# happyjin/Gaussian_process

Measured on AMD Instinct MI355X. Metric: GP-fit+predict sec and achieved fp64 TFLOP/s, N=65536 d=8, 1/2/4/8 MI355X, higher is better.
Workload: dtype f64; 1 GPU; GP fit+predict N=65536 d=8 n_test=4096 (BASELINE configs[2]); N=65536, d=8, n_test=4096, partition=single GPU

## Files before the change

gaussian_process_amd/csrc/gemm_dma.hip:

```cpp
#include <algorithm>
#include <cstdlib>
#include <type_traits>

#include "gpmi_internal.h"
#include "gpmi_plan.h"
#include <atomic>
#include <mutex>

namespace gpmi {

typedef double d4 __attribute__((ext_vector_type(4)));
typedef double d2 __attribute__((ext_vector_type(2)));

#define GPMI_LDS __attribute__((address_space(3)))
#define GPMI_GLB __attribute__((address_space(1)))
#define GPMI_CONST __attribute__((address_space(4)))

struct GemmDmaDev {
    double* C;
    const double* A;
    const double* B;
    int64_t ldc, lda, ldb;
    int Tm, Tn;
    int nchunks;
    int lower;
    int64_t diag_off;
    const int32_t* row_ncols;
    int row_block_tiles;
    const int64_t* b_block_off;
    int b_block_tiles;
    int S, logS, SM, SN, tri, nsuper;
    int pair;
    int sprefix[DMA_MAX_SM + 1];
    unsigned long long* stamps;
    int dbg;
    struct PersistSlot* slot;
    int nblocks;
};

struct PersistSlot {
    unsigned ctr[8];
    unsigned done;
    unsigned pad[7];
};

template <class PT>
__device__ __forceinline__ bool dma_block_to_tile(const PT& p, int b, int& ti, int& tj) {
    return plan_block_to_tile(p, b, ti, tj);
}

__device__ __forceinline__ bool dma_map_tile(const GemmDmaDev& p, int& ti, int& tj) {
    return dma_block_to_tile(p, blockIdx.x, ti, tj);
}

constexpr int DMA_TM = PLAN_TILE, DMA_TN = PLAN_TILE;
template <class PT>
__device__ __forceinline__ bool dma_tile_live(const PT& p, int ti, int tj) {
    return plan_tile_live(p, ti, tj, p.row_ncols);
}
constexpr int DMA_STAGE_SLOTS = (DMA_TM + DMA_TN) * 8;
constexpr int DMA_STAGES = 3;

constexpr unsigned TICKET_NONE = 0xFFFFFFFFu;

template <class PT>
__device__ __forceinline__ unsigned ticket_draw(const PT& p, int xcd) {
    const unsigned per = (unsigned)p.nblocks >> 3;
#pragma unroll 1
    for (int t = 0; t < 8; ++t) {
        const int x = (xcd + t) & 7;
        if (t && __hip_atomic_load(&p.slot->ctr[x], __ATOMIC_RELAXED, __HIP_MEMORY_SCOPE_AGENT) >= per) continue;
        const unsigned w = atomicAdd(&p.slot->ctr[x], 1u);
        if (w < per) return w * 8u + (unsigned)x;
    }
    return TICKET_NONE;
}

template <int MI, bool DBG, bool TICKET = false>
__device__ __forceinline__ void gemm_nt_dma_body(const GemmDmaDev& p) {
    constexpr int NWAVES = 16 / MI;
    constexpr int DPW = 32 / NWAVES;
    constexpr int RPW = DMA_TM / NWAVES;
    constexpr int NFR = MI + 4;
    const int dbg = DBG ? p.dbg : 0;
    extern __shared__ __attribute__((aligned(16))) char smem_raw[];
    const int tid = threadIdx.x;
    volatile GPMI_LDS int* mbox = (volatile GPMI_LDS int*)(smem_raw + DMA_STAGES * DMA_STAGE_SLOTS * 16);
    unsigned blk = blockIdx.x, nxt_blk = TICKET_NONE;
    int par = 0;
    if constexpr (TICKET) {
        if (tid == 0) mbox[0] = (int)ticket_draw(p, (int)(blockIdx.x & 7));
        __syncthreads();
        blk = (unsigned)__builtin_amdgcn_readfirstlane(mbox[0]);
        par = 1;
    }
  for (;;) {
    int ti = 0, tj = 0;
    bool live;
    if constexpr (TICKET) {
        if (blk == TICKET_NONE) break;
        live = dma_block_to_tile(p, (int)blk, ti, tj) && dma_tile_live(p, ti, tj);
        live = __builtin_amdgcn_readfirstlane(live ? 1 : 0) != 0;
        ti = __builtin_amdgcn_readfirstlane(ti);
        tj = __builtin_amdgcn_readfirstlane(tj);
    } else {
        live = dma_map_tile(p, ti, tj) && dma_tile_live(p, ti, tj);
        if (!live) return;
    }
   if (live) {
    unsigned long long st0 = 0, st1 = 0, st2 = 0, st3 = 0;
    if (DBG && (dbg & 16)) st0 = clock64();
    const int lane = tid & 63;
    const int wave = __builtin_amdgcn_readfirstlane(tid >> 6);
    const int wr = (wave >> 1) * (16 * MI);
    const int wc = (wave & 1) * 64;
    const int fr = lane & 15;
    const int fg = lane >> 4;

// ... 172 lines not shown
            if (!live) nxt_blk = ticket_draw(p, (int)(blockIdx.x & 7));
            mbox[par] = (int)nxt_blk;
        }
        __syncthreads();
        blk = (unsigned)__builtin_amdgcn_readfirstlane(mbox[par]);
        par ^= 1;
    }
  }
    if constexpr (TICKET) {
        if (tid == 0) {
            __threadfence();
            const unsigned old = atomicAdd(&p.slot->done, 1u);
            if (old == gridDim.x - 1) {
#pragma unroll
                for (int x = 0; x < 8; ++x) p.slot->ctr[x] = 0;
                p.slot->done = 0;
                __threadfence();
            }
        }
    }
}

template <int MI, bool DBG>
__global__ __launch_bounds__(1024 / MI, (MI == 4) ? 2 : 3) void gemm_nt_dma_kernel(const GemmDmaDev p) {
    gemm_nt_dma_body<MI, DBG>(p);
}

__global__ __launch_bounds__(512, 3) void chol_trailing_update_dma_kernel(const GemmDmaDev p) {
    gemm_nt_dma_body<2, false>(p);
}

constexpr int TALL_TM = 2 * DMA_TM;
constexpr int TALL_STAGE_SLOTS = (TALL_TM + DMA_TN) * 8;
constexpr int TALL_STAGES = 2;
constexpr size_t TALL_LDS = (size_t)TALL_STAGES * TALL_STAGE_SLOTS * 16;
static_assert(TALL_LDS == (size_t)DMA_STAGES * DMA_STAGE_SLOTS * 16, "the tall form keeps the LDS footprint");

template <bool DBG>
__device__ __forceinline__ void gemm_nt_dma_tall_body(const GemmDmaDev& p) {
    constexpr int DPW = 6;
    const int dbg = DBG ? p.dbg : 0;
    extern __shared__ __attribute__((aligned(16))) char smem_raw[];
    const int tid = threadIdx.x;
    int ti = 0, tj = 0;
    if (!dma_block_to_tile(p, blockIdx.x, ti, tj)) return;
    bool l0, l1;
    plan_pair_live(p, ti, tj, p.row_ncols, l0, l1);
    ti = __builtin_amdgcn_readfirstlane(ti);
    tj = __builtin_amdgcn_readfirstlane(tj);
    const bool live0 = __builtin_amdgcn_readfirstlane(l0 ? 1 : 0) != 0;
    const bool live1 = __builtin_amdgcn_readfirstlane(l1 ? 1 : 0) != 0;
    if (!live0 && !live1) return;
    unsigned long long st0 = 0, st1 = 0, st2 = 0, st3 = 0;
    if (DBG && (dbg & 16)) st0 = clock64();
    const int lane = tid & 63;
    const int wave = __builtin_amdgcn_readfirstlane(tid >> 6);
    const bool mine = (wave >> 2) ? live1 : live0;
    const int wr = (wave >> 1) * 64;
    const int wc = (wave & 1) * 64;
    const int fr = lane & 15;
    const int fg = lane >> 4;

    const int drow = lane >> 3;
    const int dkp = (lane & 7) ^ (drow & 7);
    const int arow = 32 * wave - ((ti + 1 >= p.Tm && wave >= 4) ? DMA_TM : 0);
    const double* a_row = p.A + ((int64_t)ti * DMA_TM + arow) * p.lda;
    int64_t b_row0 = (int64_t)tj * DMA_TN * p.ldb;
    if (p.b_block_off) {
        const int blk = tj / p.b_block_tiles;
        b_row0 = p.b_block_off[blk] + (int64_t)(tj - blk * p.b_block_tiles) * DMA_TN * p.ldb;
    }
    const double* b_row = p.B + b_row0 + (int64_t)(16 * wave) * p.ldb;
    const unsigned a_lane = (unsigned)((drow * p.lda + dkp * 2) * 8);
    const unsigned b_lane = (unsigned)((drow * p.ldb + dkp * 2) * 8);
    const int64_t a_step = 8 * p.lda, b_step = 8 * p.ldb;
    GPMI_LDS char* lds = (GPMI_LDS char*)smem_raw;
    const int a_dst = (32 * wave) * 128;
    const int b_dst = TALL_TM * 128 + (16 * wave) * 128;
    auto issue_dma_one = [&](int chunk, int q) {
        GPMI_LDS char* base = lds + (chunk & 1) * (TALL_STAGE_SLOTS * 16);
        const int k0 = chunk * 16;
        unsigned off = q < 4 ? a_lane : b_lane;
        asm volatile("" : "+v"(off));
        if (q < 4)
            __builtin_amdgcn_global_load_lds((const GPMI_GLB void*)((const char*)(a_row + q * a_step + k0) + off),
                                             (GPMI_LDS void*)(base + a_dst + q * 1024), 16, 0, 0);
        else
            __builtin_amdgcn_global_load_lds((const GPMI_GLB void*)((const char*)(b_row + (q - 4) * b_step + k0) + off),
                                             (GPMI_LDS void*)(base + b_dst + (q - 4) * 1024), 16, 0, 0);
    };

    const int x7 = fr & 7;
    const int sl0 = fr * 8 + (fg ^ x7);
    const int sl1 = fr * 8 + ((4 + fg) ^ x7);
    const d2* smem = reinterpret_cast<const d2*>(smem_raw);
    auto read_a = [&](int chunk, int half, int i) -> d2 {
        return smem[(chunk & 1) * TALL_STAGE_SLOTS + (wr + 16 * i) * 8 + (half ? sl1 : sl0)];
    };
    auto read_b = [&](int chunk, int half, int j) -> d2 {
        return smem[(chunk & 1) * TALL_STAGE_SLOTS + TALL_TM * 8 + (wc + 16 * j) * 8 + (half ? sl1 : sl0)];
    };

    d4 acc[4][4];
#pragma unroll
    for (int i = 0; i < 4; ++i)
#pragma unroll
        for (int j = 0; j < 4; ++j) acc[i][j] = d4{0., 0., 0., 0.};
    const int nch = p.nchunks;

#define GPMI_MFMA_X(FA, FB, T) acc[(T) >> 2][(T) & 3] = __builtin_amdgcn_mfma_f64_16x16x4f64(FA[(T) >> 2].x, FB[(T) & 3].x, acc[(T) >> 2][(T) & 3], 0, 0, 0)
#define GPMI_MFMA_Y(FA, FB, T) acc[(T) >> 2][(T) & 3] = __builtin_amdgcn_mfma_f64_16x16x4f64(FA[(T) >> 2].y, FB[(T) & 3].y, acc[(T) >> 2][(T) & 3], 0, 0, 0)
#define GPMI_FENCE() __builtin_amdgcn_sched_barrier(0)
    auto kloop = [&](auto live_tag) {
        constexpr bool LIVE = decltype(live_tag)::value;
        d2 fa[4], fb0[4], fb1[4];
#pragma unroll
        for (int q = 0; q < DPW; ++q) issue_dma_one(0, q);
        if (nch > 1) {
#pragma unroll
            for (int q = 0; q < DPW; ++q) issue_dma_one(1, q);
            asm volatile("s_waitcnt vmcnt(6)" ::: "memory");
        } else {
            asm volatile("s_waitcnt vmcnt(0)" ::: "memory");
        }
        __builtin_amdgcn_s_barrier();
        if constexpr (LIVE) {
#pragma unroll
            for (int i = 0; i < 4; ++i) fa[i] = read_a(0, 0, i);
#pragma unroll
            for (int j = 0; j < 4; ++j) fb0[j] = read_b(0, 0, j);
        }
        if (DBG && (dbg & 16)) st1 = clock64();
        auto quarter0 = [&]() {
            if constexpr (LIVE) {
#pragma unroll
                for (int t = 0; t < 16; ++t) GPMI_MFMA_X(fa, fb0, t);
                GPMI_FENCE();
            }
        };
        auto step = [&](int c) {
            const bool more2 = (c + 2 < nch) && !(dbg & 1);
            if constexpr (LIVE) {
#pragma unroll
                for (int q = 0; q < 8; ++q) {
                    GPMI_MFMA_Y(fa, fb0, 2 * q);
                    GPMI_MFMA_Y(fa, fb0, 2 * q + 1);
                    GPMI_FENCE();
                    if (q & 1) fa[q >> 1] = read_a(c, 1, q >> 1);
                    else fb1[q >> 1] = read_b(c, 1, q >> 1);
                    GPMI_FENCE();
                }
#pragma unroll
                for (int t = 0; t < 8; ++t) GPMI_MFMA_X(fa, fb1, t);
                GPMI_FENCE();
            }
            if (!(dbg & 2)) {
                asm volatile("s_waitcnt vmcnt(0)\n\ts_waitcnt lgkmcnt(0)" ::: "memory");
                __builtin_amdgcn_s_barrier();
            }
            GPMI_FENCE();
            if constexpr (LIVE) {
#pragma unroll
                for (int t = 8; t < 16; ++t) {
                    GPMI_MFMA_X(fa, fb1, t);
                    GPMI_FENCE();
                    if (more2 && t - 8 < DPW) issue_dma_one(c + 2, t - 8);
                    GPMI_FENCE();
                }
#pragma unroll
                for (int q = 0; q < 8; ++q) {
                    GPMI_MFMA_Y(fa, fb1, 2 * q);
                    GPMI_MFMA_Y(fa, fb1, 2 * q + 1);
                    GPMI_FENCE();
                    if (q & 1) fa[q >> 1] = read_a(c + 1, 0, q >> 1);
                    else fb0[q >> 1] = read_b(c + 1, 0, q >> 1);
                    GPMI_FENCE();
                }
            } else if (more2) {
#pragma unroll
                for (int q = 0; q < DPW; ++q) issue_dma_one(c + 2, q);
            }
        };
        quarter0();
        for (int c = 0; c + 1 < nch; ++c) {
            step(c);
            quarter0();
        }
        step(nch - 1);
    };
    if (mine) kloop(std::true_type{});
    else kloop(std::false_type{});
#undef GPMI_MFMA_X
#undef GPMI_MFMA_Y
#undef GPMI_FENCE
    if (!mine) return;

    if (DBG && (dbg & 16)) st2 = clock64();
    double* Cg = p.C + ((int64_t)ti * DMA_TM + wr) * p.ldc + (int64_t)tj * DMA_TN + wc;
    auto c_ptr = [&](int i, int j, int v) { return Cg + (int64_t)(16 * i + 4 * v + fg) * p.ldc + 16 * j + fr; };
    if (DBG && (dbg & 8)) {
        double t = 0.;
#pragma unroll
        for (int i = 0; i < 4; ++i)
#pragma unroll
            for (int j = 0; j < 4; ++j) t += acc[i][j][0] + acc[i][j][1] + acc[i][j][2] + acc[i][j][3];
        if (t == 123.456) Cg[0] = t;
        return;
    }
    double cv[2][4][4];
    auto load_band = [&](int i) {
#pragma unroll
        for (int j = 0; j < 4; ++j)
#pragma unroll
            for (int v = 0; v < 4; ++v) cv[i & 1][j][v] = *c_ptr(i, j, v);
    };
    auto store_band = [&](int i) {
#pragma unroll
        for (int j = 0; j < 4; ++j)
#pragma unroll
            for (int v = 0; v < 4; ++v) *c_ptr(i, j, v) = cv[i & 1][j][v] - acc[i][j][v];
    };
    load_band(0);
    if (DBG && (dbg & 16)) {
        asm volatile("s_waitcnt vmcnt(0)" ::: "memory");
        st3 = clock64();
    }
    store_band(0);
    load_band(1);
    load_band(2);
    store_band(1);
    load_band(3);
    store_band(2);
    store_band(3);
    if (DBG && (dbg & 16)) {
        asm volatile("s_waitcnt vmcnt(0)" ::: "memory");
        const unsigned long long st4 = clock64();
        if (lane == 0 && blockIdx.x < 4096) {
            unsigned long long* o = p.stamps + ((size_t)blockIdx.x * 4 + (wave & 3)) * 4;
            o[0] = st1 - st0; o[1] = st2 - st1; o[2] = st3 - st2; o[3] = st4 - st3;
        }
    }
}

template <bool DBG>
__global__ __launch_bounds__(512) __attribute__((amdgpu_num_vgpr(192))) void gemm_nt_dma_tall_kernel(const GemmDmaDev p) {
    gemm_nt_dma_tall_body<DBG>(p);
}
__global__ __launch_bounds__(512) __attribute__((amdgpu_num_vgpr(192))) void chol_trailing_update_dma256_kernel(const GemmDmaDev p) {
    gemm_nt_dma_tall_body<false>(p);
}

__global__ __launch_bounds__(512, 3) void gemm_nt_dma_ticket_kernel(const GemmDmaDev p) {
    gemm_nt_dma_body<2, false, true>(p);
}
__global__ __launch_bounds__(512, 3) void chol_trailing_update_ticket_kernel(const GemmDmaDev p) {
    gemm_nt_dma_body<2, false, true>(p);
}

template <int ROLE>
__device__ __forceinline__ void gemm_nt_dma_persist_body(const GemmDmaDev& p) {
    constexpr int MI = 2, DPW = 4, RPW = 16, NFR = 6, NT = 8, NSLOT = 4;
    constexpr int RING = DMA_STAGES * DMA_STAGE_SLOTS * 16;
    extern __shared__ __attribute__((aligned(16))) char smem_raw[];
    volatile GPMI_LDS int* mbox = (volatile GPMI_LDS int*)(smem_raw + RING);
    const int tid = threadIdx.x;
    const int lane = tid & 63;
    const int wave = __builtin_amdgcn_readfirstlane(tid >> 6);
    const int wr = (wave >> 1) * (16 * MI);
    const int wc = (wave & 1) * 64;
    const int fr = lane & 15;
    const int fg = lane >> 4;
    const int drow = lane >> 3;
    const int dkp = (lane & 7) ^ (drow & 7);
    const int xcd = blockIdx.x & 7;
    const int nch = p.nchunks;
    const int64_t ldc = p.ldc;
    GPMI_LDS char* lds = (GPMI_LDS char*)smem_raw;
    const int a_dst = (RPW * wave) * 128;
    const int b_dst = DMA_TM * 128 + (RPW * wave) * 128;
    const unsigned c_lane = (unsigned)((fg * ldc + fr) * 8);

    auto kernarg = [&]() -> const GPMI_CONST GemmDmaDev* {
        const GPMI_CONST GemmDmaDev* pp = (const GPMI_CONST GemmDmaDev*)__builtin_amdgcn_kernarg_segment_ptr();
        asm volatile("" : "+s"(pp));
        return pp;
    };
    auto uniform_ptr = [](const void* q) -> uintptr_t {
        const uintptr_t u = reinterpret_cast<uintptr_t>(q);
        const unsigned lo = (unsigned)__builtin_amdgcn_readfirstlane((int)(u & 0xffffffffu));
        const unsigned hi = (unsigned)__builtin_amdgcn_readfirstlane((int)(u >> 32));
        return ((uintptr_t)hi << 32) | lo;
    };
    struct TileRef { const double* d[DPW]; GPMI_GLB char* c; };
    auto resolve = [&](unsigned b, TileRef& t) -> bool {
        const GPMI_CONST GemmDmaDev* pp = kernarg();
        int ti, tj;
        if (!dma_block_to_tile(*pp, (int)b, ti, tj)) return false;
        if (!dma_tile_live(*pp, ti, tj)) return false;
        ti = __builtin_amdgcn_readfirstlane(ti);
        tj = __builtin_amdgcn_readfirstlane(tj);
        t.d[0] = pp->A + ((int64_t)ti * DMA_TM + RPW * wave + drow) * pp->lda + dkp * 2;
        t.d[1] = t.d[0] + 8 * pp->lda;
        int64_t b_row0 = (int64_t)tj * DMA_TN * pp->ldb;
        if (pp->b_block_off) {
            const int blk = tj / pp->b_block_tiles;
            b_row0 = pp->b_block_off[blk] + (int64_t)(tj - blk * pp->b_block_tiles) * DMA_TN * pp->ldb;
        }
        t.d[2] = pp->B + b_row0 + (int64_t)(RPW * wave + drow) * pp->ldb + dkp * 2;
        t.d[3] = t.d[2] + 8 * pp->ldb;
        double* tc = pp->C + ((int64_t)ti * DMA_TM + wr) * pp->ldc + (int64_t)tj * DMA_TN + wc;
        t.c = (GPMI_GLB char*)uniform_ptr(tc);
        return true;
    };
    auto draw = [&]() -> unsigned {
        const GPMI_CONST GemmDmaDev* pp = kernarg();
        return ticket_draw(*pp, xcd);
    };
    auto past_end = [&](unsigned b) -> bool { return b == TICKET_NONE; };
    auto scalar_flag = [](bool f) -> bool { return __builtin_amdgcn_readfirstlane(f ? 1 : 0) != 0; };
    auto draw_sync = [&](TileRef& t) -> bool {
        for (;;) {
            if (tid == 0) mbox[0] = (int)draw();
            __syncthreads();
            const unsigned w = (unsigned)__builtin_amdgcn_readfirstlane(mbox[0]);
// ... 268 lines not shown
        for (int j = 0; j < 2; ++j)
#pragma unroll
            for (int v = 0; v < 4; ++v) cv[i][j][v] = *c_ptr(i, j, v);
#pragma unroll
    for (int i = 0; i < 2; ++i)
#pragma unroll
        for (int j = 0; j < 2; ++j)
#pragma unroll
            for (int v = 0; v < 4; ++v) *c_ptr(i, j, v) = cv[i][j][v] - acc[i][j][v];
}

hipError_t launch_gemm_nt_small(hipStream_t s, const GemmArgs& a, const GemmRoute& r) {
    GemmSmallDev p;
    p.C = a.C; p.A = a.A; p.B = a.B; p.ldc = a.ldc; p.lda = a.lda; p.ldb = a.ldb;
    p.Tm = (int)(a.M / SM_T); p.Tn = (int)(a.N / SM_T); p.nchunks = (int)(a.K / 16);
    p.lower = a.lower; p.diag_off = a.diag_off;
    static PerDeviceOnce once;
    const hipError_t ea = once.run([&]() -> hipError_t {
        return hipFuncSetAttribute((const void*)gemm_nt_small_kernel<8>, hipFuncAttributeMaxDynamicSharedMemorySize, (int)(8 * GEMM_SMALL_STAGE));
    });
    if (ea != hipSuccess) return ea;
    if (r.kernel == GemmKernel::Small3) hipLaunchKernelGGL(gemm_nt_small_kernel<3>, dim3(r.grid), dim3(256), r.lds, s, p);
    else hipLaunchKernelGGL(gemm_nt_small_kernel<8>, dim3(r.grid), dim3(256), r.lds, s, p);
    return hipGetLastError();
}

struct PersistPool {
    static constexpr int SLOTS = 16384;
    PersistSlot* base = nullptr;
    int groups = 0;
    std::atomic<unsigned> head{0};
    PersistSlot* next() { return base + (head.fetch_add(1, std::memory_order_relaxed) % SLOTS); }
};

static PersistPool* persist_pool() {
    static std::mutex mu;
    static PersistPool pools[16];
    int dev = 0;
    if (hipGetDevice(&dev) != hipSuccess || dev < 0 || dev >= 16) return nullptr;
    PersistPool& pl = pools[dev];
    std::lock_guard<std::mutex> lock(mu);
    if (!pl.base) {
        hipDeviceProp_t prop;
        if (hipGetDeviceProperties(&prop, dev) != hipSuccess) return nullptr;
        void* q = nullptr;
        if (hipMalloc(&q, sizeof(PersistSlot) * PersistPool::SLOTS) != hipSuccess) return nullptr;
        if (hipMemset(q, 0, sizeof(PersistSlot) * PersistPool::SLOTS) != hipSuccess) { (void)hipFree(q); return nullptr; }
        pl.groups = (prop.multiProcessorCount / 8) * 8;
        if (pl.groups < 8) { (void)hipFree(q); return nullptr; }
        const void* fns[] = {(const void*)gemm_nt_dma_persist_kernel, (const void*)chol_trailing_update_persist_kernel,
                             (const void*)gemm_nt_dma_ticket_kernel, (const void*)chol_trailing_update_ticket_kernel};
        for (const void* f : fns)
            if (hipFuncSetAttribute(f, hipFuncAttributeMaxDynamicSharedMemorySize,
                                    (int)(DMA_STAGES * DMA_STAGE_SLOTS * 16 + 16)) != hipSuccess) { (void)hipFree(q); return nullptr; }
        pl.base = static_cast<PersistSlot*>(q);
    }
    return &pl;
}

int gemm_resident_groups() {
    const PersistPool* pool = persist_pool();
    return pool ? pool->groups : 0;
}

static_assert((size_t)DMA_STAGES * DMA_STAGE_SLOTS * 16 == GEMM_DMA_LDS && TALL_LDS == GEMM_TALL_LDS && TALL_LDS == GEMM_DMA_LDS,
              "gpmi_route.h sizes the rings of the launches; one opt-in size serves both forms");

hipError_t launch_gemm_nt_dma(hipStream_t s, const GemmArgs& a, const GemmRoute& r) {
    const TilePlan& plan = r.plan;
    GemmDmaDev p;
    p.C = a.C; p.A = a.A; p.B = a.B;
    p.ldc = a.ldc; p.lda = a.lda; p.ldb = a.ldb;
    p.Tm = plan.Tm; p.Tn = plan.Tn;
    p.nchunks = (int)(a.K / 16);
    p.lower = a.lower; p.diag_off = a.diag_off;
    p.row_ncols = a.row_ncols; p.row_block_tiles = plan.row_block_tiles;
    p.b_block_off = a.b_block_off;
    p.b_block_tiles = a.b_block_off ? (int)(a.b_block_rows / 128) : 1;
    p.S = plan.S; p.logS = plan.logS; p.SM = plan.SM; p.SN = plan.SN; p.tri = plan.tri; p.nsuper = plan.nsuper;
    p.pair = plan.pair;
    if (plan.tri == 2) std::copy(plan.sprefix, plan.sprefix + plan.SM + 1, p.sprefix);
    p.dbg = tuning().gemm_dbg & 0xff;
    p.stamps = tuning().gemm_stamps;
    p.slot = nullptr;
    p.nblocks = plan.nblocks;
    static PerDeviceOnce once;
    const hipError_t ea = once.run([&]() -> hipError_t {
        const void* fns[] = {(const void*)gemm_nt_dma_kernel<4, false>, (const void*)gemm_nt_dma_kernel<4, true>,
                             (const void*)gemm_nt_dma_kernel<2, false>, (const void*)gemm_nt_dma_kernel<2, true>,
                             (const void*)chol_trailing_update_dma_kernel, (const void*)gemm_nt_dma_tall_kernel<false>,
                             (const void*)gemm_nt_dma_tall_kernel<true>, (const void*)chol_trailing_update_dma256_kernel};
        for (const void* f : fns) {
            const hipError_t e = hipFuncSetAttribute(f, hipFuncAttributeMaxDynamicSharedMemorySize, (int)GEMM_DMA_LDS);
            if (e != hipSuccess) return e;
        }
        return hipSuccess;
    });
    if (ea != hipSuccess) return ea;
    if (r.kernel >= GemmKernel::Persist) {
        PersistPool* pool = persist_pool();
        if (!pool) return hipErrorInvalidValue;
        p.slot = pool->next();
    }
    const dim3 grid(r.grid);
    switch (r.kernel) {
        case GemmKernel::Ticket: hipLaunchKernelGGL(gemm_nt_dma_ticket_kernel, grid, dim3(512), r.lds, s, p); break;
        case GemmKernel::TicketTrail: hipLaunchKernelGGL(chol_trailing_update_ticket_kernel, grid, dim3(512), r.lds, s, p); break;
        case GemmKernel::Persist: hipLaunchKernelGGL(gemm_nt_dma_persist_kernel, grid, dim3(512), r.lds, s, p); break;
        case GemmKernel::PersistTrail: hipLaunchKernelGGL(chol_trailing_update_persist_kernel, grid, dim3(512), r.lds, s, p); break;
        case GemmKernel::Tall: hipLaunchKernelGGL(gemm_nt_dma_tall_kernel<false>, grid, dim3(512), r.lds, s, p); break;
        case GemmKernel::TallProbe: hipLaunchKernelGGL(gemm_nt_dma_tall_kernel<true>, grid, dim3(512), r.lds, s, p); break;
        case GemmKernel::TallTrail: hipLaunchKernelGGL(chol_trailing_update_dma256_kernel, grid, dim3(512), r.lds, s, p); break;
        case GemmKernel::Dma8: hipLaunchKernelGGL((gemm_nt_dma_kernel<2, false>), grid, dim3(512), r.lds, s, p); break;
        case GemmKernel::Dma8Probe: hipLaunchKernelGGL((gemm_nt_dma_kernel<2, true>), grid, dim3(512), r.lds, s, p); break;
        case GemmKernel::Dma8Trail: hipLaunchKernelGGL(chol_trailing_update_dma_kernel, grid, dim3(512), r.lds, s, p); break;
        case GemmKernel::Dma4: hipLaunchKernelGGL((gemm_nt_dma_kernel<4, false>), grid, dim3(256), r.lds, s, p); break;
        case GemmKernel::Dma4Probe: hipLaunchKernelGGL((gemm_nt_dma_kernel<4, true>), grid, dim3(256), r.lds, s, p); break;
        default: return hipErrorInvalidValue;
    }
    return hipGetLastError();
}

}
```

gaussian_process_amd/csrc/gpmi_api.hip:

```cpp
#include "gpmi_ctx.h"

using namespace gpmi;

namespace gpmi {
thread_local std::string g_err;

static thread_local Tuning t_dev_tuning;
static thread_local const Tuning* t_tuning = nullptr;
const Tuning& tuning() { return t_tuning ? *t_tuning : t_dev_tuning; }
TuneScope::TuneScope(const Tuning* t) : prev(t_tuning) { t_tuning = t; }
TuneScope::~TuneScope() { t_tuning = prev; }
static thread_local Sharing t_sharing;
Sharing& sharing() { return t_sharing; }

int ard_rescale_train(gpmi_ctx* c) {
    if (!c->ard()) return GPMI_OK;
    HIP_TRY(c->Xz.ensure((size_t)c->N * c->d * 8));
    HIP_TRY(launch_scale_inputs(c->stream, c->X.as<double>(), c->ard_rdev.as<double>(), c->N, c->d, c->Xz.as<double>()));
    HIP_TRY(hipStreamSynchronize(c->stream));
    box_scale(c->boxX, c->ard_r, c->boxZ);
    return GPMI_OK;
}
int ard_rescale_test(gpmi_ctx* c) {
    if (!c->ard()) return GPMI_OK;
// ... 15 lines not shown
    int n = 0;
    hipError_t e = hipGetDeviceCount(&n);
    if (e != hipSuccess) { *count = 0; return fail_runtime(e, "hipGetDeviceCount"); }
    *count = n;
    return GPMI_OK;
}

int gpmi_ctx_create(int device, gpmi_ctx** out) {
    if (!out) return fail_arg("gpmi_ctx_create: null out pointer");
    *out = nullptr;
    int n = 0;
    HIP_TRY(hipGetDeviceCount(&n));
    if (device < 0 || device >= n) return fail_arg("gpmi_ctx_create: no such device");
    HIP_TRY(hipSetDevice(device));
    gpmi_ctx* c = new gpmi_ctx();
    c->device = device;
    int prio_lo = 0, prio_hi = 0;
    (void)hipDeviceGetStreamPriorityRange(&prio_lo, &prio_hi);
    hipError_t e = hipStreamCreateWithPriority(&c->stream, hipStreamNonBlocking, prio_lo);
    if (e != hipSuccess) { delete c; return fail_runtime(e, "hipStreamCreate"); }
    e = hipStreamCreateWithPriority(&c->pstream, hipStreamNonBlocking, prio_hi);
    if (e != hipSuccess) { (void)hipStreamDestroy(c->stream); delete c; return fail_runtime(e, "hipStreamCreate"); }
    const char* env;
    if ((env = getenv("GPMI_NB"))) c->nb = std::max<int64_t>(128, atoll(env) / 128 * 128);
    if ((env = getenv("GPMI_LD_PAD"))) c->ld_pad = std::max<int64_t>(0, atoll(env) / 2 * 2);
    if ((env = getenv("GPMI_LOOKAHEAD"))) c->lookahead = atoi(env) ? 1 : 0;
    *out = c;
    return GPMI_OK;
}

int gpmi_ctx_destroy(gpmi_ctx* c) {
    if (!c) return GPMI_OK;
    for (gpmi_ctx* l : c->lane_ctx) (void)gpmi_ctx_destroy(l);
    c->lane_ctx.clear();
    (void)hipSetDevice(c->device);
    (void)hipStreamSynchronize(c->stream);
    for (DevBuf* b : {&c->X, &c->y, &c->A, &c->info, &c->red, &c->Xs, &c->V, &c->P, &c->vec, &c->dense,
                       &c->U, &c->Kn, &c->gpart, &c->cov_a, &c->cov_b, &c->cov_out, &c->flag, &c->vside,
                       &c->Xz, &c->Xsz, &c->ard_rdev, &c->gsum, &c->app, &c->spareA, &c->rem, &c->lap, &c->lap_part, &c->lap_out, &c->sm, &c->sm_part, &c->sm_E, &c->sm_B, &c->sm_out, &c->loov, &c->loow,
                       &c->sp_Zraw, &c->sp_Z, &c->sp_L, &c->sp_B, &c->sp_W, &c->sp_q, &c->sp_vec, &c->sp_part, &c->sp_scr, &c->sp_info, &c->sp_pred,
                       &c->sp_g0, &c->sp_g1, &c->sp_g2, &c->sp_gE, &c->sp_gpart, &c->sp_gvec})
        b->release();
    for (auto e : c->ev_pool) (void)hipEventDestroy(e);
    (void)hipStreamDestroy(c->stream);
    (void)hipStreamDestroy(c->pstream);
    delete c;
    return GPMI_OK;
}

static int set_tuning_option(Tuning& t, const char* name, int64_t value) {
    if (!strcmp(name, "gemm_small_tiles")) {
        t.gemm_small_tiles = value ? 1 : 0;
    } else if (!strcmp(name, "trsm_wave")) {
        t.trsm_wave = value ? 1 : 0;
    } else if (!strcmp(name, "gemm_small_dma")) {
        t.gemm_small_dma = value ? 1 : 0;
    } else if (!strcmp(name, "gemm_persist")) {
        t.gemm_persist = value ? 1 : 0;
    } else if (!strcmp(name, "gemm_ticket")) {
        if (value < 0 || value > 2) return fail_arg("gemm_ticket must be 0 (off), 1 (trailing updates under lookahead) or 2 (every launch)");
        t.gemm_ticket = (int)value;
    } else if (!strcmp(name, "gemm_balance")) {
        t.gemm_balance = value ? 1 : 0;
    } else if (!strcmp(name, "trsv_vinv")) {
        if (value < 0 || value > 2) return fail_arg("trsv_vinv must be 0 (16 x 16 rounds), 1 (one launch per block) or 2 (one launch)");
        t.trsv_vinv = (int)value;
    } else if (!strcmp(name, "panel_fused")) {
        t.panel_fused = value ? 1 : 0;
    } else if (!strcmp(name, "rbf_blocks")) {
        if (value < 1 || value > (1 << 24)) return fail_arg("rbf_blocks must be in 1..2^24");
        t.rbf_blocks = (int)value;
    } else if (!strcmp(name, "gemm_dma_waves")) {
        if (value != 4 && value != 8) return fail_arg("gemm_dma_waves must be 4 or 8");
        t.gemm_dma_waves = (int)value;
    } else if (!strcmp(name, "gemm_tall")) {
        if (value < 0 || value > 1) return fail_arg("gemm_tall must be 0 (128 x 128 blocks) or 1 (256 x 128 blocks for large launches)");
        t.gemm_tall = (int)value;
    } else if (!strcmp(name, "tall_min_tiles")) {
        if (value < 0 || value > (1 << 30)) return fail_arg("tall_min_tiles must be in 0..2^30");
        t.tall_min_tiles = (int)value;
    } else if (!strcmp(name, "tall_min_tiles_slack")) {
        if (value < 0 || value > (1 << 30)) return fail_arg("tall_min_tiles_slack must be in 0..2^30");
        t.tall_min_tiles_slack = (int)value;
    } else if (!strcmp(name, "gemm_dma")) {
        t.gemm_use_dma = value ? 1 : 0;
    } else {
        return -1;
    }
    return GPMI_OK;
}

int gpmi_set_option(gpmi_ctx* c, const char* name, int64_t value) {
    if (!c || !name) return fail_arg("gpmi_set_option: null argument");
    if (!strcmp(name, "nb")) {
        if (value != 0 && (value < 128 || value % 128)) return fail_arg("nb must be 0 (auto) or a positive multiple of 128");
        c->nb = value;
    } else if (!strcmp(name, "ld_pad")) {
        if (value < 0 || value % 2) return fail_arg("ld_pad must be even and >= 0");
        c->ld_pad = value;
        c->res.drop_fit();
    } else if (!strcmp(name, "timing")) {
        c->timing = value ? 1 : 0;
    } else if (!strcmp(name, "lookahead")) {
        c->lookahead = value ? 1 : 0;
    } else if (!strcmp(name, "la_min")) {
        if (value < 0) return fail_arg("la_min must be >= 0");
        c->la_min = value;
    } else if (!strcmp(name, "shallow_min")) {
        if (value < 0) return fail_arg("shallow_min must be >= 0");
        c->shallow_min = value;
    } else if (!strcmp(name, "sparse_slab")) {
        if (value < 0) return fail_arg("sparse_slab must be >= 0 (0: by size)");
        c->sparse_slab = value;
    } else if (!strcmp(name, "reserve")) {
        if (value < 0) return fail_arg("reserve must be >= 0 (points that gpmi_append may add in place)");
        c->reserve = value;
    } else if (!strcmp(name, "append_skinny")) {
        if (value < -1 || value > 1) return fail_arg("append_skinny must be -1 (by size), 0 (never) or 1 (whenever allowed)");
        c->append_skinny = (int)value;
    } else if (!strcmp(name, "remove_keep_spare")) {
        c->remove_keep_spare = value ? 1 : 0;
        if (!c->remove_keep_spare) {
            HIP_TRY(hipSetDevice(c->device));
            c->spareA.release();
        }
    } else if (!strcmp(name, "lanes")) {
        if (value < 0 || value > 8) return fail_arg("lanes must be 0 (by size) .. 8");
        c->lanes = (int)value;
    } else {
        const int rc = set_tuning_option(c->tune, name, value);
        if (rc < 0) return fail_arg("gpmi_set_option: unknown option");
        return rc;
    }
    return GPMI_OK;
}

int gpmi_dev_set_option(const char* name, int64_t value) {
    if (!name) return fail_arg("gpmi_dev_set_option: null argument");
    const int rc = set_tuning_option(t_dev_tuning, name, value);
    if (rc < 0) return fail_arg("gpmi_dev_set_option: unknown option");
    return rc;
}

int gpmi_set_kernel(gpmi_ctx* c, int kind, double p0, double p1) {
    if (!c) return fail_arg("gpmi_set_kernel: null context");
    if (kind < 0 || kind == 3 || kind > 6)
        return fail_arg("gpmi_set_kernel: kind must be 0 (rbf), 1 (linear), 2 (periodic) or 4, 5, 6 (Matern nu = 1/2, 3/2, 5/2)");
    if (kind == 2 && (!(p0 != 0.0) || !(p1 != 0.0))) return fail_arg("gpmi_set_kernel: period and lengthscale must be non-zero");
    c->kind = kind; c->kp0 = p0; c->kp1 = p1;
    c->res.drop_fit();
    return GPMI_OK;
}

int gpmi_set_kernel_params(gpmi_ctx* c, int kind, const double* params, int nparams) {
    if (!c || !params) return fail_arg("gpmi_set_kernel_params: null argument");
    if (kind != 3) {
        if (kind < 0 || kind > 6 || nparams != 2) return fail_arg("gpmi_set_kernel_params: kinds 0-2 and 4-6 take 2 parameters");
        return gpmi_set_kernel(c, kind, params[0], params[1]);
    }
    if (nparams != 11) return fail_arg("gpmi_set_kernel_params: the CO2 composite kernel takes 11 hyper-parameters (CO2_example.py:86-89)");
    if (!(params[1] != 0.0) || !(params[3] != 0.0) || !(params[4] != 0.0) || !(params[6] != 0.0) || !(params[7] != 0.0) ||
        !(params[9] != 0.0))
        return fail_arg("gpmi_set_kernel_params: theta_2, 4, 5, 7, 8, 10 divide and must be non-zero");
    c->kind = 3;
    for (int i = 0; i < 11; ++i) c->kpv[i] = params[i];
    c->res.drop_fit();
// ... 491 lines not shown
```

gaussian_process_amd/csrc/gpmi_internal.h:

```cpp
#pragma once
#include <hip/hip_runtime.h>
#include <stdint.h>

#include <cmath>
#include <mutex>

#include "gpmi_kroute.h"
#include "gpmi_route.h"

namespace gpmi {

constexpr int TILE = 128;
constexpr int IB = 64;

struct Tuning : GemmTuning {
    int trsm_wave = 1;
    int rbf_blocks = 16384;
    int trsv_vinv = 2;
    int panel_fused = 1;
    unsigned long long* gemm_stamps = nullptr;
    unsigned long long* panel_stamps = nullptr;
};
const Tuning& tuning();
struct TuneScope {
    const Tuning* prev;
    explicit TuneScope(const Tuning* t);
    ~TuneScope();
};
Sharing& sharing();
struct SharingScope {
    const Sharing prev;
    explicit SharingScope(Sharing s) : prev(sharing()) { sharing() = s; }
    ~SharingScope() { sharing() = prev; }
};

struct PerDeviceOnce {
    std::mutex mu;
    uint64_t done = 0;
    template <class F> hipError_t run(F fn) {
        int dev = 0;
        hipError_t e = hipGetDevice(&dev);
        if (e != hipSuccess) return e;
        std::lock_guard<std::mutex> lock(mu);
        if (dev < 64 && ((done >> dev) & 1)) return hipSuccess;
        e = fn();
        if (e == hipSuccess && dev < 64) done |= (uint64_t)1 << dev;
        return e;
    }
};

struct GemmArgs {
    double* C;
    const double* A;
    const double* B;
    int64_t ldc, lda, ldb;
    int64_t M, N, K;
    int mode = 0;
    int lower = 0;
    int64_t diag_off = 0;
    const int32_t* row_ncols = nullptr;
    int row_block_tiles = 1;
    const int32_t* row_ncols_host = nullptr;
    int row_bands = 0;
    int role = 0;
    const int64_t* b_block_off = nullptr;
    int64_t b_block_rows = 0;
};
inline GemmArgs gemm_minus(double* C, int64_t ldc, const double* A, int64_t lda, const double* B, int64_t ldb, int64_t M,
                           int64_t N, int64_t K) {
    GemmArgs g;
    g.C = C; g.A = A; g.B = B;
    g.ldc = ldc; g.lda = lda; g.ldb = ldb;
    g.M = M; g.N = N; g.K = K;
    return g;
}
inline GemmArgs gemm_minus_lower(double* C, int64_t ldc, const double* A, int64_t lda, const double* B, int64_t ldb,
                                 int64_t M, int64_t N, int64_t K, int64_t diag_off) {
    GemmArgs g = gemm_minus(C, ldc, A, lda, B, ldb, M, N, K);
    g.lower = 1; g.diag_off = diag_off;
    return g;
}
GemmRoute gemm_nt_route(const GemmArgs& a);
hipError_t launch_gemm_nt(hipStream_t s, const GemmArgs& a, const GemmRoute& r);
inline hipError_t launch_gemm_nt(hipStream_t s, const GemmArgs& a) { return launch_gemm_nt(s, a, gemm_nt_route(a)); }
double gemm_nt_algorithmic_flops(const GemmArgs& a, int64_t real_rows);
hipError_t launch_gemm_nt_dma(hipStream_t s, const GemmArgs& a, const GemmRoute& r);
hipError_t launch_gemm_nt_small(hipStream_t s, const GemmArgs& a, const GemmRoute& r);
int gemm_resident_groups();
double gemm_nt_flops(const GemmArgs& a);

hipError_t launch_potf2_64(hipStream_t s, double* A, int64_t ld, int64_t col_offset,
                           int64_t* info_dev);
hipError_t launch_trsm_rlt64(hipStream_t s, const double* L, int64_t ldl, double* X, int64_t ldx,
                             int64_t m);

hipError_t launch_potrf128(hipStream_t s, double* A, int64_t ld, int64_t col_offset, int64_t* info_dev);

hipError_t launch_trsm128(hipStream_t s, const double* L, int64_t ldl, double* X, int64_t ldx, int64_t m);

hipError_t launch_border_sweep(hipStream_t s, const double* L, int64_t ldl, int64_t ncols, double* X, int64_t ldx,
                               int64_t rows);

// ... 128 lines not shown
```

Before: 69.06 TFLOP/s.

## Prefetch C tile rows into LDS during final k-chunks of tall GEMM

In the tall DMA GEMM kernel, the last two k-chunk steps now issue global-to-LDS DMA loads of the first C rows into the freed stage buffers. The epilogue reads those rows from LDS and overlaps the remaining global loads of C with the stores. It also makes the DMA source address scalar and restructures the C pointer lane offsets to reduce address arithmetic. The goal is to hide the C read-modify-write latency in the epilogue, at the cost of more complex sync and a new tuning flag, enabled by default.

```diff
diff --git a/gaussian_process_amd/csrc/gemm_dma.hip b/gaussian_process_amd/csrc/gemm_dma.hip
--- a/gaussian_process_amd/csrc/gemm_dma.hip
+++ b/gaussian_process_amd/csrc/gemm_dma.hip
@@ -34,6 +34,7 @@
     int sprefix[DMA_MAX_SM + 1];
     unsigned long long* stamps;
     int dbg;
+    int c_ring;
     struct PersistSlot* slot;
     int nblocks;
 };
@@ -372,12 +373,10 @@
         const int k0 = chunk * 16;
         unsigned off = q < 4 ? a_lane : b_lane;
         asm volatile("" : "+v"(off));
-        if (q < 4)
-            __builtin_amdgcn_global_load_lds((const GPMI_GLB void*)((const char*)(a_row + q * a_step + k0) + off),
-                                             (GPMI_LDS void*)(base + a_dst + q * 1024), 16, 0, 0);
-        else
-            __builtin_amdgcn_global_load_lds((const GPMI_GLB void*)((const char*)(b_row + (q - 4) * b_step + k0) + off),
-                                             (GPMI_LDS void*)(base + b_dst + (q - 4) * 1024), 16, 0, 0);
+        const char* src = q < 4 ? (const char*)(a_row + q * a_step + k0) : (const char*)(b_row + (q - 4) * b_step + k0);
+        asm volatile("" : "+s"(src));
+        __builtin_amdgcn_global_load_lds((const GPMI_GLB void*)(src + off),
+                                         (GPMI_LDS void*)(base + (q < 4 ? a_dst + q * 1024 : b_dst + (q - 4) * 1024)), 16, 0, 0);
     };
 
     const int x7 = fr & 7;
@@ -398,6 +397,21 @@
         for (int j = 0; j < 4; ++j) acc[i][j] = d4{0., 0., 0., 0.};
     const int nch = p.nchunks;
 
+    double* Cg = p.C + ((int64_t)ti * DMA_TM + wr) * p.ldc + (int64_t)tj * DMA_TN + wc;
+    const bool cring = p.c_ring && nch >= 3 && !(dbg & (1 | 8));
+    constexpr int C_RING_ROWS = 2 * DPW;
+    constexpr int C_RING_WAVE = C_RING_ROWS * 64 * 8;
+    static_assert(8 * C_RING_WAVE <= TALL_STAGE_SLOTS * 16, "the eight regions lie inside a stage");
+    auto issue_c_dma = [&](int c, int q) {
+        unsigned l;
+        asm volatile("v_mbcnt_lo_u32_b32 %0, -1, 0\n\tv_mbcnt_hi_u32_b32 %0, -1, %0" : "=v"(l));
+        const unsigned off = ((l >> 5) * (unsigned)p.ldc + 2 * (l & 31)) * 8;
+        const int row = (c + 1 == nch ? C_RING_ROWS : 0) + 2 * q;
+        __builtin_amdgcn_global_load_lds((const GPMI_GLB void*)((const char*)(Cg + (int64_t)row * p.ldc) + off),
+                                         (GPMI_LDS void*)(lds + (c & 1) * (TALL_STAGE_SLOTS * 16) + wave * C_RING_WAVE + q * 1024),
+                                         16, 0, 0);
+    };
+
 #define GPMI_MFMA_X(FA, FB, T) acc[(T) >> 2][(T) & 3] = __builtin_amdgcn_mfma_f64_16x16x4f64(FA[(T) >> 2].x, FB[(T) & 3].x, acc[(T) >> 2][(T) & 3], 0, 0, 0)
 #define GPMI_MFMA_Y(FA, FB, T) acc[(T) >> 2][(T) & 3] = __builtin_amdgcn_mfma_f64_16x16x4f64(FA[(T) >> 2].y, FB[(T) & 3].y, acc[(T) >> 2][(T) & 3], 0, 0, 0)
 #define GPMI_FENCE() __builtin_amdgcn_sched_barrier(0)
@@ -428,8 +442,10 @@
                 GPMI_FENCE();
             }
         };
-        auto step = [&](int c) {
-            const bool more2 = (c + 2 < nch) && !(dbg & 1);
+        auto step = [&](int c, auto tail_tag) {
+            constexpr bool TAIL = decltype(tail_tag)::value;
+            const bool more2 = !TAIL && !(dbg & 1);
+            const bool cpre = TAIL && cring;
             if constexpr (LIVE) {
 #pragma unroll
                 for (int q = 0; q < 8; ++q) {
@@ -455,6 +471,7 @@
                     GPMI_MFMA_X(fa, fb1, t);
                     GPMI_FENCE();
                     if (more2 && t - 8 < DPW) issue_dma_one(c + 2, t - 8);
+                    if (cpre && t - 8 < DPW) issue_c_dma(c, t - 8);
                     GPMI_FENCE();
                 }
 #pragma unroll
@@ -472,11 +489,15 @@
             }
         };
         quarter0();
-        for (int c = 0; c + 1 < nch; ++c) {
-            step(c);
+        for (int c = 0; c + 2 < nch; ++c) {
+            step(c, std::false_type{});
             quarter0();
         }
-        step(nch - 1);
+        if (nch > 1) {
+            step(nch - 2, std::true_type{});
+            quarter0();
+        }
+        step(nch - 1, std::true_type{});
     };
     if (mine) kloop(std::true_type{});
     else kloop(std::false_type{});
@@ -486,8 +507,12 @@
     if (!mine) return;
 
     if (DBG && (dbg & 16)) st2 = clock64();
-    double* Cg = p.C + ((int64_t)ti * DMA_TM + wr) * p.ldc + (int64_t)tj * DMA_TN + wc;
-    auto c_ptr = [&](int i, int j, int v) { return Cg + (int64_t)(16 * i + 4 * v + fg) * p.ldc + 16 * j + fr; };
+    const unsigned c_lane = ((unsigned)fg * (unsigned)p.ldc + (unsigned)fr) * 8;
+    auto c_ptr = [&](int i, int j, int v) {
+        unsigned off = c_lane;
+        asm volatile("" : "+v"(off));
+        return (double*)((char*)(Cg + (int64_t)(16 * i + 4 * v) * p.ldc + 16 * j) + off);
+    };
     if (DBG && (dbg & 8)) {
         double t = 0.;
 #pragma unroll
@@ -497,39 +522,71 @@
         if (t == 123.456) Cg[0] = t;
         return;
     }
-    double cv[2][4][4];
-    auto load_band = [&](int i) {
+    auto write_stamps = [&]() {
+        if (DBG && (dbg & 16)) {
+            asm volatile("s_waitcnt vmcnt(0)" ::: "memory");
+            const unsigned long long st4 = clock64();
+            if (lane == 0 && blockIdx.x < 4096) {
+                unsigned long long* o = p.stamps + ((size_t)blockIdx.x * 4 + (wave & 3)) * 4;
+                o[0] = st1 - st0; o[1] = st2 - st1; o[2] = st3 - st2; o[3] = st4 - st3;
+            }
+        }
+    };
+    if (cring) {
+        double cr[6][4], cl[4];
+        auto load_group = [&](int g, double* d) {
+#pragma unroll
+            for (int j = 0; j < 4; ++j) d[j] = *c_ptr(g >> 2, j, g & 3);
+        };
+        auto store_group = [&](int g, const double* s) {
+#pragma unroll
+            for (int j = 0; j < 4; ++j) *c_ptr(g >> 2, j, g & 3) = s[j] - acc[g >> 2][j][g & 3];
+        };
+#pragma unroll
+        for (int g = 6; g < 12; ++g) load_group(g, cr[g - 6]);
+        __builtin_amdgcn_sched_barrier(0);
+        asm volatile("s_waitcnt vmcnt(24)" ::: "memory");
+        if (DBG && (dbg & 16)) st3 = clock64();
+        const GPMI_LDS char* cl0 = lds + wave * C_RING_WAVE + fg * 512 + fr * 8;
+        const GPMI_LDS char* clA = cl0 + (nch & 1) * (TALL_STAGE_SLOTS * 16);
+        const GPMI_LDS char* clB = cl0 + ((nch & 1) ^ 1) * (TALL_STAGE_SLOTS * 16);
+#pragma unroll
+        for (int g = 0; g < 6; ++g) {
+#pragma unroll
+            for (int j = 0; j < 4; ++j)
+                cl[j] = *(const GPMI_LDS double*)((g < 3 ? clA : clB) + (g % 3) * 4 * 512 + j * 128);
+            store_group(g, cl);
+            __builtin_amdgcn_sched_barrier(0);
+        }
+        double cr2[4][4];
+#pragma unroll
+        for (int g = 12; g < 16; ++g) load_group(g, cr2[g - 12]);
+#pragma unroll
+        for (int g = 6; g < 12; ++g) store_group(g, cr[g - 6]);
+        __builtin_amdgcn_sched_barrier(0);
+#pragma unroll
+        for (int g = 12; g < 16; ++g) store_group(g, cr2[g - 12]);
+        write_stamps();
+        return;
+    }
+    double cv[4][4];
+#pragma unroll
+    for (int i = 0; i < 4; ++i) {
 #pragma unroll
         for (int j = 0; j < 4; ++j)
 #pragma unroll
-            for (int v = 0; v < 4; ++v) cv[i & 1][j][v] = *c_ptr(i, j, v);
-    };
-    auto store_band = [&](int i) {
+            for (int v = 0; v < 4; ++v) cv[j][v] = *c_ptr(i, j, v);
+        if (DBG && (dbg & 16) && i == 0) {
+            asm volatile("s_waitcnt vmcnt(0)" ::: "memory");
+            st3 = clock64();
+        }
 #pragma unroll
         for (int j = 0; j < 4; ++j)
 #pragma unroll
-            for (int v = 0; v < 4; ++v) *c_ptr(i, j, v) = cv[i & 1][j][v] - acc[i][j][v];
-    };
-    load_band(0);
-    if (DBG && (dbg & 16)) {
-        asm volatile("s_waitcnt vmcnt(0)" ::: "memory");
-        st3 = clock64();
-    }
-    store_band(0);
-    load_band(1);
-    load_band(2);
-    store_band(1);
-    load_band(3);
-    store_band(2);
-    store_band(3);
-    if (DBG && (dbg & 16)) {
-        asm volatile("s_waitcnt vmcnt(0)" ::: "memory");
-        const unsigned long long st4 = clock64();
-        if (lane == 0 && blockIdx.x < 4096) {
-            unsigned long long* o = p.stamps + ((size_t)blockIdx.x * 4 + (wave & 3)) * 4;
-            o[0] = st1 - st0; o[1] = st2 - st1; o[2] = st3 - st2; o[3] = st4 - st3;
-        }
-    }
+            for (int v = 0; v < 4; ++v) *c_ptr(i, j, v) = cv[j][v] - acc[i][j][v];
+        __builtin_amdgcn_sched_barrier(0);
+    }
+    write_stamps();
 }
 
 template <bool DBG>
@@ -964,6 +1021,7 @@
     if (plan.tri == 2) std::copy(plan.sprefix, plan.sprefix + plan.SM + 1, p.sprefix);
     p.dbg = tuning().gemm_dbg & 0xff;
     p.stamps = tuning().gemm_stamps;
+    p.c_ring = tuning().tall_c_ring && (reinterpret_cast<uintptr_t>(a.C) & 15) == 0 && (a.ldc & 1) == 0;
     p.slot = nullptr;
     p.nblocks = plan.nblocks;
     static PerDeviceOnce once;
diff --git a/gaussian_process_amd/csrc/gpmi_api.hip b/gaussian_process_amd/csrc/gpmi_api.hip
--- a/gaussian_process_amd/csrc/gpmi_api.hip
+++ b/gaussian_process_amd/csrc/gpmi_api.hip
@@ -121,6 +121,8 @@
     } else if (!strcmp(name, "tall_min_tiles_slack")) {
         if (value < 0 || value > (1 << 30)) return fail_arg("tall_min_tiles_slack must be in 0..2^30");
         t.tall_min_tiles_slack = (int)value;
+    } else if (!strcmp(name, "tall_c_ring")) {
+        t.tall_c_ring = value ? 1 : 0;
     } else if (!strcmp(name, "gemm_dma")) {
         t.gemm_use_dma = value ? 1 : 0;
     } else {
diff --git a/gaussian_process_amd/csrc/gpmi_internal.h b/gaussian_process_amd/csrc/gpmi_internal.h
--- a/gaussian_process_amd/csrc/gpmi_internal.h
+++ b/gaussian_process_amd/csrc/gpmi_internal.h
@@ -18,6 +18,7 @@
     int rbf_blocks = 16384;
     int trsv_vinv = 2;
     int panel_fused = 1;
+    int tall_c_ring = 1;
     unsigned long long* gemm_stamps = nullptr;
     unsigned long long* panel_stamps = nullptr;
 };
```

After: 69.68 TFLOP/s (median of 6 runs). No clear change (+0.9%).
